# nash169/manifold-gp

Hardware: AMD Instinct MI355X
Metric: CG-solve wall-time + SpMV HBM GB/s, N=60k RMNIST graph (higher is better)
Workload: dtype f32; 1 GPU; C3 RMNIST-like N=60000 d=784 k=50 nu=2 randomwalk; nodes=60000, edges=1777442, nnz_padded=3667592, rhs_columns=1, system=A = I + noise*outputscale*Q, Q=(2nu/kappa^2 I + L)^nu x D, solver=CG on A (Chronopoulos-Gear, one hipGraph per solve)

## Files before the change

include/mgp_hip.h:

```cpp
#ifndef MGP_HIP_H
#define MGP_HIP_H

#include <stddef.h>
#include <stdint.h>

#ifdef __cplusplus
extern "C" {
#endif

#define MGP_OK 0
#define MGP_ERR_ARG (-1)
#define MGP_ERR_WORKSPACE (-2)
#define MGP_ERR_UNSUPPORTED (-3)
#define MGP_ERR_NOT_CONVERGED (-4)
#define MGP_ERR_KNN_AMBIGUOUS (-5)
#define MGP_ERR_TIMEOUT (-6)

#define MGP_PAD 4

int mgp_version(void);
int mgp_device_info(int* cu_count, int* wave_size, size_t* hbm_bytes);

size_t mgp_knn_workspace_bytes(int64_t N, int64_t n, int d, int k);
int mgp_knn_search(const float* db, int64_t N, int d, const float* q, int64_t n, int k,
// ... 129 lines not shown

typedef struct {
  float tol;
  int32_t max_iter;
  int32_t min_iter;
  int32_t stop_mode;
  int32_t check_every;
  int32_t use_graph;
  int32_t max_refine;
} mgp_cg_params_t;

size_t mgp_cg_workspace_bytes(const mgp_operator_t* op, int C);
int mgp_cg_set_decide_in_update(int on);
int mgp_cg_set_complex_shift(int on);
int mgp_cg_plan_is_complex_shift(void* plan);
int mgp_cg_set_fold_update(int on);
int mgp_cg_plan_is_folded(void* plan);
int mgp_cg_set_reduce_once(int on);
int mgp_cg_set_update_quads(int on);
int mgp_cg_set_poll_spin(int spins);
int mgp_cg_set_init_free(int on);
int mgp_cg_plan_create(const mgp_operator_t* op, int C, const float* minv,
                       const mgp_cg_params_t* params, void* work, size_t work_bytes, void* stream,
                       void** plan_out);
int mgp_cg_plan_solve(void* plan, const float* B, float* X, int32_t* iters, float* resid,
                      int32_t* status);
int mgp_cg_plan_rebind(void* plan, const mgp_operator_t* op, const float* minv);
float* mgp_cg_plan_x(void* plan);
double* mgp_cg_plan_x64(void* plan);
int mgp_cg_plan_last_applies(void* plan);
// ... 179 lines not shown
```

manifold_gp_amd/_lib.py:

```python
import ctypes
import os
import threading
from ctypes import (POINTER, Structure, byref, c_double, c_float, c_int, c_int32, c_int64, c_size_t,
                    c_uint64, c_void_p)

import torch

_HERE = os.path.dirname(os.path.abspath(__file__))
LIB_PATH = os.path.join(_HERE, "libmgp_hip.so")
_LIB = None
_LOCK = threading.Lock()

MGP_ERRORS = {
    -1: "MGP_ERR_ARG (null pointer / bad size / bad enum)",
    -2: "MGP_ERR_WORKSPACE (work buffer too small)",
    -3: "MGP_ERR_UNSUPPORTED",
    -4: "MGP_ERR_NOT_CONVERGED",
    -5: "MGP_ERR_KNN_AMBIGUOUS",
}


class MgpError(RuntimeError):
    def __init__(self, fn, code):
        self.code = code
# ... 57 lines not shown
    "mgp_spmm_dot_blocks_csr": (c_int, [POINTER(CsrT), c_int]),
    "mgp_spmm_set_tile_mode": (c_int, [c_int]),
    "mgp_spmm_set_tile_loop_mode": (c_int, [c_int]),
    "mgp_spmm_set_tile_small_mode": (c_int, [c_int]),
    "mgp_spmm_set_tile_wide_mode": (c_int, [c_int]),
    "mgp_spmm_set_dict_mode": (c_int, [c_int]),
    "mgp_spmm_set_mt_mode": (c_int, [c_int]),
    "mgp_spmm_kernel_choice": (c_int, [POINTER(CsrT), c_int, c_int, c_int64]),
    "mgp_spmm_mt_fill": (c_int, [c_int64, _P, _P, _P, _P, _P, _P, c_int64, _P, _P, _P]),
    "mgp_spmm_timing_begin": (c_int, [c_int]),
    "mgp_spmm_timing_end": (c_int, [POINTER(c_float), POINTER(c_int)]),
    "mgp_spmm_set_v4_mode": (c_int, [c_int]),
    "mgp_cg_set_decide_in_update": (c_int, [c_int]),
    "mgp_cg_set_complex_shift": (c_int, [c_int]),
    "mgp_cg_plan_is_complex_shift": (c_int, [_P]),
    "mgp_cg_set_fold_update": (c_int, [c_int]),
    "mgp_cg_plan_is_folded": (c_int, [_P]),
    "mgp_cg_set_reduce_once": (c_int, [c_int]),
    "mgp_cg_set_update_quads": (c_int, [c_int]),
    "mgp_cg_set_poll_spin": (c_int, [c_int]),
    "mgp_cg_set_init_free": (c_int, [c_int]),
    "mgp_host_symeig": (c_int, [c_int, _P, _P, _P]),
    "mgp_lanczos_set_bound_mode": (c_int, [c_int]),
    "mgp_blz_workspace_bytes": (c_size_t, [c_int64, c_int, c_int]),
    "mgp_blz_begin": (c_int, [_P, c_int64, c_int, c_int, _P, c_size_t, _P]),
    "mgp_blz_q": (c_void_p, [c_int64, c_int, c_int, c_int, _P, c_size_t]),
    "mgp_blz_step": (c_int, [_P, c_int64, c_int, c_int, c_int, _P, c_size_t, _P]),
    "mgp_blz_end": (c_int, [c_int64, c_int, c_int, POINTER(c_float), POINTER(c_float), _P, c_size_t, _P]),
    "mgp_lanczos_tridiag_block_workspace_bytes": (c_size_t, [POINTER(OperatorT), c_int, c_int]),
    "mgp_lanczos_tridiag_block": (c_int, [POINTER(OperatorT), _P, c_int, c_int, POINTER(c_float), POINTER(c_float), _P,
# ... 237 lines not shown
```

manifold_gp_amd/csrc/cg.hip:

```cpp
#include <math.h>
#include <chrono>
#include <mutex>
#include <new>
#include <vector>
#include <string.h>
#include <algorithm>
#include "mgp_common.h"
#include "mgp_internal.h"
#include "cg_rule.h"
#include "cg_policy.h"
#include "cg_handoff.h"

namespace {

#ifndef MGP_LAB_UPD
#define MGP_LAB_UPD 0
#endif

typedef float mgp_cg_v4f __attribute__((ext_vector_type(4)));

struct CgArgs {
  int64_t n;
  int C, TC, TS;
  float *x, *r, *u, *w, *p, *s;
// ... 647 lines not shown
  const mgp_cg_v4f* y4;
  const float* pd4;
  int nbs4;
  float sigma;
  float* pd_g;
  float* sc;
};

__device__ __forceinline__ float2 cx_mul(float2 a, float2 b) { return make_float2(a.x * b.x - a.y * b.y, a.x * b.y + a.y * b.x); }
__device__ __forceinline__ float2 cx_div(float2 a, float2 b) {
  const float d = b.x * b.x + b.y * b.y;
  if (!(d > 0.f)) return make_float2(0.f, 0.f);
  return make_float2((a.x * b.x + a.y * b.y) / d, (a.y * b.x - a.x * b.y) / d);
}

__global__ __launch_bounds__(kBlock) void cx_init_kernel(CgArgs a, CxArgs c, const float* __restrict__ B) {
  __shared__ float sh_o[kBlock / 64];
  const int tid = threadIdx.x, lane = tid & 63, wave = tid >> 6;
  const int lb = mgp_xcd_block(blockIdx.x, gridDim.x);
  const int64_t r0 = (int64_t)lb * a.rows_per_block;
  int64_t r1 = r0 + a.rows_per_block;
  if (r1 > a.n) r1 = a.n;
  if (blockIdx.x == 0 && tid == 0) { a.state[0] = 0; a.state[1] = 0; a.state[2] = 0; }
  float g = 0.f;
  for (int64_t r = r0 + tid; r < r1; r += kBlock) {
    const float b = B[r];
    c.z[r] = make_float2(0.f, 0.f);
    c.r[r] = make_float2(b, 0.f);
    c.p[r] = make_float2(0.f, 0.f);
    c.s[r] = make_float2(0.f, 0.f);
    c.u4[r] = mgp_cg_v4f{b, 0.f, b, 0.f};
    c.w4[r] = mgp_cg_v4f{b, 0.f, 0.f, b};
    a.x[r] = 0.f;
    g = fmaf(b, b, g);
  }
  g = mgp_wave_sum(g);
  if (lane == 0) sh_o[wave] = g;
  __syncthreads();
  if (tid == 0) {
    const float t = (sh_o[0] + sh_o[1]) + (sh_o[2] + sh_o[3]);
    float* dst = c.pd_g + 4 * (int64_t)lb;
    dst[0] = t; dst[1] = 0.f; dst[2] = t; dst[3] = t;
  }
}

__global__ __launch_bounds__(kBlock) void cx_update_kernel(CgArgs a, CxArgs c) {
  __shared__ float sh_w[kBlock / 64][8];
  __shared__ float sh_o[kBlock / 64][4];
  __shared__ int sh_state[2];
  const int tid = threadIdx.x, lane = tid & 63, wave = tid >> 6;
  const int st_it = a.state[0], st_done = a.state[1];
  const int lb = mgp_xcd_block(blockIdx.x, gridDim.x);
  const int64_t r0 = (int64_t)lb * a.rows_per_block;
  int64_t r1 = r0 + a.rows_per_block;
  if (r1 > a.n) r1 = a.n;
  float t[8] = {0.f, 0.f, 0.f, 0.f, 0.f, 0.f, 0.f, 0.f};
  mgp_cg_v4f gv[2][kC1GammaSlots];
#pragma unroll
  for (int h = 0; h < 2; ++h) {
#pragma unroll
// ... 66 lines not shown
  const CgStop st = cg_stop(1, 0, a.max_iter + 1, a.tol, it, rel);
  const int done = st.done;
  if (blockIdx.x == 0 && tid == 0) {
    c.sc[4 * par + 0] = gamma.x; c.sc[4 * par + 1] = gamma.y;
    c.sc[4 * par + 2] = alpha.x; c.sc[4 * par + 3] = alpha.y;
    if (it == 1) c.sc[8] = bb;
    a.resid[0] = rel;
    if (done) cg_publish(a.state, a.host_state, a.host_resid, &rel, 1, it, st.status);
  }
  if (done) return;
  float ngr = 0.f, ngi = 0.f, nrr = 0.f, nee = 0.f;
  constexpr int U = 4;
  const int64_t rf = r0 + tid;
  for (int64_t rb = rf; rb < r1; rb += (int64_t)U * kBlock) {
    float2 uo[U], po[U], so[U], zo[U];
    mgp_cg_v4f yo[U];
#pragma unroll
    for (int k = 0; k < U; ++k) {
      const int64_t r = rb + (int64_t)k * kBlock;
      const int64_t rc = r < r1 ? r : rf;
      uo[k] = c.r[rc]; po[k] = c.p[rc]; so[k] = c.s[rc]; zo[k] = c.z[rc]; yo[k] = c.y4[rc];
    }
#pragma unroll
    for (int k = 0; k < U; ++k) {
      const int64_t r = rb + (int64_t)k * kBlock;
      if (r < r1) {
        const float2 u = uo[k];
        const float2 w = make_float2(u.x - c.sigma * yo[k].y, u.y + c.sigma * yo[k].x);
        const float e = u.x + c.sigma * yo[k].y;
        const float2 bp = cx_mul(beta, po[k]), bs = cx_mul(beta, so[k]);
        const float2 pn = make_float2(u.x + bp.x, u.y + bp.y);
        const float2 sn = make_float2(w.x + bs.x, w.y + bs.y);
        const float2 ap = cx_mul(alpha, pn), as = cx_mul(alpha, sn);
        const float2 zn = make_float2(zo[k].x + ap.x, zo[k].y + ap.y);
        const float2 rn = make_float2(u.x - as.x, u.y - as.y);
        c.p[r] = pn; c.s[r] = sn; c.z[r] = zn; c.r[r] = rn;
        a.x[r] = zo[k].x;
        c.u4[r] = mgp_cg_v4f{rn.x, rn.y, rn.x, rn.y};
        c.w4[r] = mgp_cg_v4f{rn.x, rn.y, rn.y, rn.x};
        ngr += rn.x * rn.x - rn.y * rn.y;
        ngi += 2.f * rn.x * rn.y;
        nrr += rn.x * rn.x + rn.y * rn.y;
        nee = fmaf(e, e, nee);
      }
    }
  }
  ngr = mgp_wave_sum(ngr); ngi = mgp_wave_sum(ngi); nrr = mgp_wave_sum(nrr); nee = mgp_wave_sum(nee);
  if (lane == 0) { sh_o[wave][0] = ngr; sh_o[wave][1] = ngi; sh_o[wave][2] = nrr; sh_o[wave][3] = nee; }
  __syncthreads();
  if (tid == 0) {
    float* dst = c.pd_g + 4 * ((int64_t)par * a.nbv + lb);
    dst[0] = (sh_o[0][0] + sh_o[1][0]) + (sh_o[2][0] + sh_o[3][0]);
    dst[1] = (sh_o[0][1] + sh_o[1][1]) + (sh_o[2][1] + sh_o[3][1]);
    dst[2] = (sh_o[0][2] + sh_o[1][2]) + (sh_o[2][2] + sh_o[3][2]);
// ... 152 lines not shown
  hipGraph_t graph_first = nullptr;
  hipGraphExec_t exec_first = nullptr;
  hipGraphNode_t init_node = nullptr;
  bool has_graph = false, has_first = false;
  int chunk = 0, len_first = 0;
  int last_need = 0;
  const float* patched_rhs = nullptr;
  int solves = 0;
  int64_t last_solve_ns = 0;
  int marker_seq = 0;
  bool graphs_tried = false;
  bool rebound = false;
  bool decide_in_update = false;
  CxArgs cxa{};
  mgp_operator_t opB{};
  char first_record[MGP_SPMM_RECORD_BYTES] = {};
  int32_t* host_state = nullptr;
  float* host_resid = nullptr;
  float* host_true_rel = nullptr;
  float* dev_true_rel = nullptr;
};

CgKnobs g_knobs;

CgShape cg_shape(const mgp_operator_t* op, int C, int world, bool is_dist, bool has_minv, int stop_mode) {
  CgShape sh{};
  sh.n = op->L.n; sh.world = world; sh.is_dist = is_dist; sh.C = C;
  sh.nb_loc = mgp_spmm_dot_blocks_for(&op->L, C);
  sh.nb4 = (C == 1 && !is_dist) ? mgp_spmm_dot_blocks_for(&op->L, 4) : 0;
  sh.has_minv = has_minv; sh.has_pre = op->pre != nullptr; sh.has_post = op->post != nullptr;
// ... 31 lines not shown

MgpCgStep fold_step(const CgPlan* pl) {
  const CgArgs& a = pl->args;
  MgpCgStep cs{};
  cs.r = a.r; cs.x = a.x; cs.p = a.p; cs.s = a.s; cs.us = a.us; cs.pre = a.pre;
  cs.pd_rr = a.pd_rr; cs.pd_delta = a.pd_delta; cs.nbs = a.nbs;
  cs.blk = a.gamma_old; cs.state = a.state; cs.host_state = a.host_state; cs.host_resid = a.host_resid; cs.arrive = a.arrive;
  cs.tol = a.tol; cs.max_iter = a.max_iter; cs.min_iter = a.min_iter; cs.stop_mode = a.stop_mode;
  return cs;
}

int enqueue_body(CgPlan* pl, hipStream_t st, bool decide_last = false) {
  if (pl->ch.fold)
    return mgp_operator_apply_cgstep(&pl->op, pl->args.us ? pl->args.us : pl->args.r, false, nullptr, fold_step(pl), decide_last,
                                     pl->buf.op_work, pl->buf.op_work_bytes, st);
  if (pl->ch.cx) {
    MGP_TRY(mgp_operator_apply_dist(&pl->opB, nullptr, reinterpret_cast<const float*>(pl->cxa.u4), nullptr, 4,
                                    const_cast<float*>(reinterpret_cast<const float*>(pl->cxa.y4)),
                                    reinterpret_cast<const float*>(pl->cxa.w4), pl->buf.pd4, pl->cxa.nbs4, pl->args.state + 1,
                                    pl->args.state, pl->buf.op_work4, pl->buf.op_work4_bytes, st));
    hipLaunchKernelGGL(cx_update_kernel, dim3(pl->args.nbv), dim3(kBlock), 0, st, pl->args, pl->cxa);
    MGP_LAUNCH_CHECK();
    return MGP_OK;
  }
  MGP_TRY(mgp_operator_apply_dist(&pl->op, pl->is_dist ? &pl->dist : nullptr, pl->args.u, pl->args.us, pl->C,
                                  pl->args.w, pl->args.u, pl->buf.pd_delta, pl->nb_loc, pl->args.state + 1,
                                  pl->args.state, pl->buf.op_work, pl->buf.op_work_bytes, st));
  if (pl->ch.c1_family) {
    launch_update_c1(pl, st, decide_last);
  } else {
    if (pl->args.tot) {
      hipLaunchKernelGGL(cg_reduce_kernel, dim3((unsigned)mgp_cdiv(pl->C, 4), 3), dim3(kBlock), 0, st, pl->args);
      MGP_LAUNCH_CHECK();
    }
    if (pl->ch.upd_quads) hipLaunchKernelGGL(cg_update_q_kernel<kBlock>, dim3(pl->args.nbv), dim3(kBlock), 0, st, pl->args);
    else hipLaunchKernelGGL(cg_update_kernel, dim3(pl->args.nbv), dim3(kBlock), 0, st, pl->args);
// ... 207 lines not shown
  a.tol = prm.tol; a.max_iter = prm.max_iter; a.min_iter = prm.min_iter; a.stop_mode = prm.stop_mode;
  (void)hipMemsetAsync(a.state, 0, (16 + kStampWords) * sizeof(int), pl->stream);
  MGP_HIP_TRY(hipMemsetAsync(a.arrive, 0, 9 * 32 * sizeof(int), pl->stream));
  if (b.cz) {
    CxArgs& cx = pl->cxa;
    cx.z = reinterpret_cast<float2*>(b.cz); cx.r = reinterpret_cast<float2*>(b.cr);
    cx.p = reinterpret_cast<float2*>(b.cp); cx.s = reinterpret_cast<float2*>(b.cs);
    cx.u4 = reinterpret_cast<mgp_cg_v4f*>(b.u4); cx.w4 = reinterpret_cast<mgp_cg_v4f*>(b.w4);
    cx.y4 = reinterpret_cast<const mgp_cg_v4f*>(b.y4);
    cx.pd4 = b.pd4; cx.pd_g = b.pd_g; cx.sc = b.sc;
  }
  if (ch.cx) {
    pl->opB = cx_operator(op);
    pl->cxa.nbs4 = sh.nb4;
    pl->cxa.sigma = sqrtf(sh.noise_scale);
    MGP_HIP_TRY(hipMemsetAsync(pl->cxa.sc, 0, 64 * sizeof(float), pl->stream));
  }
  const size_t rbytes = (((size_t)C * sizeof(float)) + 63) & ~size_t(63);
  if (!host_block_acquire(64 + 2 * rbytes, &pl->host_block)) { delete pl; return (int)hipErrorOutOfMemory; }
  char* hb = static_cast<char*>(pl->host_block.p);
  pl->host_state = reinterpret_cast<int32_t*>(hb);
  pl->host_resid = reinterpret_cast<float*>(hb + 64);
  pl->host_true_rel = reinterpret_cast<float*>(hb + 64 + rbytes);
  hipError_t e = hipHostGetDevicePointer((void**)&a.host_state, pl->host_state, 0);
  if (e == hipSuccess) e = hipHostGetDevicePointer((void**)&a.host_resid, pl->host_resid, 0);
  if (e == hipSuccess) e = hipHostGetDevicePointer((void**)&pl->dev_true_rel, pl->host_true_rel, 0);
  if (e != hipSuccess) { host_block_release(pl->host_block, pl->stream); delete pl; return (int)e; }
  memset(hb, 0, 64 + 2 * rbytes);

  *plan_out = pl;
  return MGP_OK;
}

extern "C" int mgp_cg_set_init_free(int on) { g_knobs.init_free = on ? 1 : 0; return MGP_OK; }
extern "C" int mgp_cg_set_poll_spin(int spins) { g_knobs.poll_spin = spins < 0 ? 0 : spins; return MGP_OK; }
extern "C" int mgp_cg_set_reduce_once(int on) { g_knobs.reduce_once = on == 2 ? 2 : (on ? 1 : 0); return MGP_OK; }
extern "C" int mgp_cg_set_update_quads(int on) { g_knobs.update_quads = on ? 1 : 0; return MGP_OK; }
extern "C" int mgp_cg_set_complex_shift(int on) { const int prev = g_knobs.complex_shift; g_knobs.complex_shift = on ? 1 : 0; return prev; }
extern "C" int mgp_cg_set_decide_in_update(int on) { const int prev = g_knobs.decide_in_update; g_knobs.decide_in_update = on ? 1 : 0; return prev; }

extern "C" int mgp_cg_set_fold_update(int on) { const int prev = g_knobs.fold_update; g_knobs.fold_update = on == 2 ? 2 : (on ? 1 : 0); return prev; }

extern "C" int mgp_cg_plan_is_folded(void* plan) {
  CgPlan* pl = static_cast<CgPlan*>(plan);
  return pl && pl->ch.fold ? 1 : 0;
}

extern "C" int mgp_cg_plan_is_complex_shift(void* plan) {
  CgPlan* pl = static_cast<CgPlan*>(plan);
  return pl && pl->ch.cx ? 1 : 0;
}

extern "C" int mgp_cg_plan_create(const mgp_operator_t* op, int C, const float* minv,
                                  const mgp_cg_params_t* params, void* work, size_t work_bytes,
                                  void* stream, void** plan_out) {
  return plan_create_impl(op, C, minv, params, nullptr, work, work_bytes, stream, plan_out);
}

extern "C" int mgp_cg_plan_rebind(void* plan, const mgp_operator_t* op, const float* minv) {
  CgPlan* pl = static_cast<CgPlan*>(plan);
  if (!pl || !op) return MGP_ERR_ARG;
  if (pl->poisoned || pl->is_dist) return MGP_ERR_UNSUPPORTED;
  const mgp_operator_t& o = pl->op;
  const bool same = op->L.n == o.L.n && op->L.ncols == o.L.ncols && op->nu == o.nu && op->form == o.form &&
                    (op->form != 3 || ((op->obs_w != nullptr) == (o.obs_w != nullptr))) &&
                    (op->pre != nullptr) == (o.pre != nullptr) && (op->post != nullptr) == (o.post != nullptr) &&
                    (minv != nullptr) == (pl->args.minv != nullptr) &&
                    (op->L.tile_ptr != nullptr) == (o.L.tile_ptr != nullptr) && op->L.tile_rows == o.L.tile_rows &&
                    op->L.tile_max_cols == o.L.tile_max_cols && op->L.tile_max_entries == o.L.tile_max_entries &&
                    (op->L.tile_rowptr != nullptr) == (o.L.tile_rowptr != nullptr) &&
                    (op->L.tile_vals != nullptr) == (o.L.tile_vals != nullptr) &&
                    (op->L.tile_rowid != nullptr) == (o.L.tile_rowid != nullptr) &&
                    (op->L.mt_img != nullptr) == (o.L.mt_img != nullptr) && op->L.mt_tiles == o.L.mt_tiles &&
                    op->L.mt_steps == o.L.mt_steps && op->L.spmv_lanes == o.L.spmv_lanes &&
                    mgp_spmm_dot_blocks_for(&op->L, pl->C) == pl->nb_loc &&
                    (!pl->ch.fold || op->pre == op->post);
  if (!same) return MGP_ERR_UNSUPPORTED;
  if (pl->ch.cx) {
    const float cc = op->noise * op->scale;
    if (!(cc > 0.f)) return MGP_ERR_UNSUPPORTED;
    pl->opB = cx_operator(op);
    if (mgp_spmm_dot_blocks_for(&pl->opB.L, 4) != pl->cxa.nbs4) return MGP_ERR_UNSUPPORTED;
    pl->cxa.sigma = sqrtf(cc);
  }
  pl->op = mgp_operator_copy(op);
  pl->args.minv = minv;
  pl->args.pre = op->pre;
  pl->rebound = true;
  return MGP_OK;
}

extern "C" size_t mgp_cg_dist_workspace_bytes(const mgp_operator_t* op_local, int C, int world) {
  if (!op_local || C <= 0 || C > kMaxC || op_local->L.n <= 0 || world < 1 || !mgp_spmv_lanes_ok(op_local->L.spmv_lanes)) return 0;
  return cg_bytes(op_local, C, world, true);
}

extern "C" int mgp_cg_plan_create_dist(const mgp_operator_t* op_local, int C, const float* minv,
// ... 6 lines not shown

static int run_cg(CgPlan* pl, const float* rhs, float* Xcopy) {
  hipStream_t st = pl->stream;
  const size_t nc = (size_t)pl->args.n * pl->C;
  pl->host_state[1] = 0;
  pl->host_state[3] = 0;
  *reinterpret_cast<volatile uint64_t*>(pl->host_state + 8) = 0;
  bool first = true;
  const auto t_begin = std::chrono::steady_clock::now();
  if (pl->rebound) refresh_graphs(pl);
  if (pl->solves++ >= 1 && !pl->graphs_tried) capture_graphs(pl);
  if (pl->has_first && !patch_first_rhs(pl, rhs)) pl->has_first = false;
  int eager_done = 0;
  if (!pl->has_first) {
    if (pl->ch.cx) {
      hipLaunchKernelGGL(cx_init_kernel, dim3(pl->args.nbv), dim3(kBlock), 0, st, pl->args, pl->cxa, rhs);
      MGP_LAUNCH_CHECK();
    } else if (pl->ch.init_free) {
      MGP_TRY(enqueue_first_body(pl, st, rhs, false));
      eager_done = 1;
    } else {
      hipLaunchKernelGGL(cg_init_kernel, dim3(pl->args.nbv), dim3(kBlock), 0, st, pl->args, rhs);
      MGP_LAUNCH_CHECK();
    }
  }
  int guard = 0;
  for (;;) {
    const bool launched_first = first && pl->has_first;
    if (launched_first) {
      ++pl->marker_seq;
      MGP_HIP_TRY(hipGraphLaunch(pl->exec_first, st));
// ... 203 lines not shown
```

manifold_gp_amd/csrc/cg_policy.h:

```cpp
#pragma once
#include <stdint.h>
#include <stddef.h>
#include "mgp_hip.h"
#include "mgp_arena.h"

constexpr int kBlock = 256;
constexpr int kMaxC = 256;
constexpr int kMaxGridVec = 512;
constexpr int kMaxPartials = 4096;
constexpr int kReduceOnceAbove = 16;
constexpr int kC1GammaSlots = 2;
constexpr int kC1DeltaSlots = 16;
constexpr int kCxDeltaSlots = 16;
#ifdef MGP_STAMP
constexpr size_t kStampWords = 1024 + 8192;
#else
constexpr size_t kStampWords = 0;
#endif

struct CgKnobs {
  int complex_shift = 1;
  int reduce_once = 1;
  int update_quads = 1;
  int poll_spin = 64;
  int init_free = 1;
  int decide_in_update = 1;
  int fold_update = 1;
};

struct CgShape {
  int64_t n;
  int world;
  bool is_dist;
  int C, nb_loc, nb4;
  bool has_minv, has_pre, has_post;
  int form, nu;
  float noise_scale;
  int stop_mode;
  bool tile_plan;
  bool pre_is_post;
  int tile_rows;
};
// ... 101 lines not shown
```

manifold_gp_amd/csrc/mgp_internal.h:

```cpp
#pragma once
#include <stddef.h>
#include <string.h>
#include <vector>
#include "mgp_hip.h"

inline mgp_operator_t mgp_operator_copy(const mgp_operator_t* op) {
  mgp_operator_t o;
  memcpy(&o, op, offsetof(mgp_operator_t, obs_w));
  o.obs_w = op->form == 3 ? op->obs_w : nullptr;
  return o;
}

inline bool mgp_spmv_lanes_ok(int lanes) {
  return lanes == 0 || lanes == 4 || lanes == 8 || lanes == 16 || lanes == 32 || lanes == 64;
}

#define MGP_SPMM_RECORD_BYTES 512
struct MgpFirst {
  float* copy_x;
  float* dot2_partials;
  int tick_reset;
  void* record;
};
struct MgpSpmmOpts {
// ... 17 lines not shown
  float* host_resid;
  int* arrive;
  float tol;
  int max_iter, min_iter, stop_mode;
  float dcoef;
  int dgamma;
};
int mgp_spmm_cgstep(const mgp_csr_t* L, const float* T, float a, float b, const float* post, float co, const MgpCgStep& cs,
                    bool decide, void* stream);
int mgp_spmm_cgstep_fits(const mgp_csr_t* L);
int mgp_operator_apply_cgstep(const mgp_operator_t* op, const float* in, bool first, void* record, const MgpCgStep& cs, bool decide,
                              void* work, size_t work_bytes, void* stream);
int mgp_spmm_fused_opts(const mgp_csr_t* L, const float* X, int C, float* Y, float a, float b, const float* pre,
                        const float* post, const float* base, float cb, float co, const float* dotw, float* dot_partials,
                        const MgpSpmmOpts& opts, void* stream);
int mgp_spmm_patch_node(void* exec, void* node, const void* record, const float* old_ptr, const float* new_ptr);
int mgp_operator_apply_first(const mgp_operator_t* op, const float* rhs, float* r_copy, float* Y, float* dot_partials,
                             float* dot2_partials, int* state, void* record, void* work, size_t work_bytes, void* stream);
int mgp_tile_plan(const mgp_csr_t* L);

int mgp_spmm_dot_blocks_for(const mgp_csr_t* L, int C);

int mgp_operator_apply_ex(const mgp_operator_t* op, const float* X, int C, float* Y, const float* dotw,
                          float* dot_partials, const int* skip, int* tick, void* work, size_t work_bytes,
                          void* stream);

int mgp_operator_apply_ex2(const mgp_operator_t* op, const float* X, const float* Xs, int C, float* Y,
                           const float* dotw, float* dot_partials, const int* skip, int* tick, void* work,
                           size_t work_bytes, void* stream);

// ... 60 lines not shown
```

manifold_gp_amd/csrc/operator.hip:

```cpp
#include <rccl/rccl.h>
#include "mgp_common.h"
#include "mgp_internal.h"

namespace {

struct Hooks {
  const float* dotw;
  float* dot_partials;
  const int* skip;
  int* tick;
  float* copy_x;
  void* record;
  float* dot2_partials;
  int tick_reset;
};

}

int mgp_dist_allgather_f32(const MgpDist* d, float* buf, int64_t count_per_rank, void* stream) {
  ncclResult_t r = ncclAllGather(buf + (int64_t)d->rank * count_per_rank, buf, (size_t)count_per_rank, ncclFloat,
                                 static_cast<ncclComm_t>(d->comm), mgp_stream(stream));
  return r == ncclSuccess ? MGP_OK : 1000 + (int)r;
}

// ... 85 lines not shown
  switch (op->form) {
    case 0:
      return q2_chain(op, d, nb_loc, X, Xs, C, Y, nullptr, 0.f, 1.f, t0, t1, &hk, stream);
    case 2:
      return q2_chain(op, d, nb_loc, X, Xs, C, Y, X, 1.f, op->noise, t0, t1, &hk, stream);
    case 3:
      return q2_chain(op, d, nb_loc, X, Xs, C, Y, X, 1.f, op->noise, t0, t1, &hk, stream, op->obs_w);
    case 1:
      MGP_TRY(q2_chain(op, d, nb_loc, X, Xs, C, ua, X, 1.f, -op->noise, t0, t1, &hk_mid, stream));
      MGP_TRY(q2_chain(op, d, nb_loc, ua, nullptr, C, ub, X, 1.f, -op->noise, t0, t1, &hk_mid, stream));
      return q2_chain(op, d, nb_loc, ub, nullptr, C, Y, nullptr, 0.f, 1.f, t0, t1, &hk, stream);
  }
  return MGP_ERR_ARG;
}

int mgp_operator_apply_first(const mgp_operator_t* op, const float* rhs, float* r_copy, float* Y, float* dot_partials,
                             float* dot2_partials, int* state, void* record, void* work, size_t work_bytes, void* stream) {
  MGP_TRY(check_op(op));
  if (!rhs || !r_copy || !Y || !dot_partials || !dot2_partials || !state || rhs == Y) return MGP_ERR_ARG;
  if (op->form != 0 && op->form != 2) return MGP_ERR_UNSUPPORTED;
  if (!work || work_bytes < 4 * mgp_align((size_t)op->L.n * sizeof(float))) return MGP_ERR_WORKSPACE;
  MgpArena ar(work, work_bytes);
  const size_t nc = (size_t)op->L.n;
  float* t0 = ar.take<float>(nc);
  float* t1 = ar.take<float>(nc);
  if (!ar.ok()) return MGP_ERR_WORKSPACE;
  const float* rv = op->nu == 1 ? rhs : r_copy;
  Hooks hk{rv, dot_partials, nullptr, state, r_copy, record, dot2_partials, 1};
  if (op->form == 0) return q2_chain(op, nullptr, 0, rhs, nullptr, 1, Y, nullptr, 0.f, 1.f, t0, t1, &hk, stream);
  return q2_chain(op, nullptr, 0, rhs, nullptr, 1, Y, rv, 1.f, op->noise, t0, t1, &hk, stream);
// ... 206 lines not shown
```

manifold_gp_amd/csrc/spmm.hip:

```cpp
#include <string.h>
#include <atomic>
#include <type_traits>
#include "mgp_common.h"
#include "mgp_internal.h"
#include "cg_rule.h"
#include "cg_handoff.h"
#include <hip/hip_ext.h>
#include <vector>

namespace {

constexpr int kBlock = 256;
constexpr int kMaxGrid = 4096;

struct SpmmArgs {
  int64_t n;
  const int32_t* rowptr;
  const int32_t* col;
  const float* vals;
  const float* diag;
  const float* X;
  float* Y;
  int C;
  float a, b;
// ... 959 lines not shown
  }
  if (p.tick && blockIdx.x == 0 && tid == 0 && !skipv) *p.tick = tickv + 1;
  if (p.dot_partials) {
    __syncthreads();
    float* red = tile_lds;
    if (sub < C4) *reinterpret_cast<mgp_v4f*>(red + (size_t)(tid >> 2) * C + 4 * sub) = dsum;
    __syncthreads();
    if (tid < C) {
      float sacc = 0.f;
      for (int r = 0; r < TR; ++r) sacc += red[r * C + tid];
      p.dot_partials[(int64_t)lb * C + tid] = sacc;
    }
  }
}

constexpr int kWideCap = 1024;
constexpr int kWideRQ = 16;

template <bool PRE, bool CBV>
__global__ __launch_bounds__(256, 2) void spmm_tile_wide_kernel(SpmmArgs p, TileArgs t, int dict_cap) {
  extern __shared__ __attribute__((aligned(16))) float tile_lds[];
  constexpr int BS = 256, TR = 64;
  const int skipv = p.skip ? *p.skip : 0;
  const int tickv = (p.tick && blockIdx.x == 0) ? *p.tick : 0;
  const int lb = mgp_xcd_block(blockIdx.x, gridDim.x);
  const int tid = threadIdx.x, sub = tid & 3;
  const int C = p.C, C4 = C >> 2;
  mgp_v4f* __restrict__ xl = reinterpret_cast<mgp_v4f*>(tile_lds);
  const mgp_v4f* __restrict__ X4 = reinterpret_cast<const mgp_v4f*>(p.X);
  const float* __restrict__ prev = p.pre;
// ... 545 lines not shown
  return (int)mgp_cdiv(ntiles, tpb);
}

static int tile_small_window(const mgp_csr_t* L) {
  const int max_q = L->tile_max_entries >> 2;
  const long budget = 40448 - (long)L->tile_max_cols * 16;
  long w = budget > 0 ? budget / 16 / 256 * 256 : 0;
  if (w < 1024) w = 1024;
  if (w > max_q) w = (max_q + 255) / 256 * 256;
  return (int)(w > 0 ? w : 256);
}
static size_t tile_small_lds_bytes(const mgp_csr_t* L, int C) {
  const size_t max_q = (size_t)(L->tile_max_entries >> 2), w = (size_t)tile_small_window(L);
  size_t b = ((size_t)L->tile_max_cols + (max_q < w ? max_q : w)) * 16;
  const size_t red = (size_t)64 * C * sizeof(float);
  return b > red ? b : red;
}

static int tile_wide_cap(const mgp_csr_t* L) {
  int cap = (L->tile_max_cols + 63) / 64 * 64;
  if (cap > kWideCap) cap = kWideCap;
  if (cap < 64) cap = 64;
  return cap;
}
static size_t tile_wide_lds_bytes(const mgp_csr_t* L) {
  const size_t b = (size_t)tile_wide_cap(L) * 64;
  return b > 4096 ? b : 4096;
}

static int dict_nv(int C) { return (C + 63) / 64; }
// ... 385 lines not shown
  const TileArgs ta = tile_args(L, pl.tiles_per_block, 0);
  const dim3 grid(pl.grid), block(256);
  hipStream_t st = mgp_stream(stream);
  auto step = [&](auto ds, auto one) {
    constexpr int DS = decltype(ds)::value;
    constexpr bool ONE = decltype(one)::value;
    if (decide) hipLaunchKernelGGL((spmv_tile_cgstep_kernel<256, DS, true, ONE>), grid, block, pl.lds, st, p, ta, cs);
    else hipLaunchKernelGGL((spmv_tile_cgstep_kernel<256, DS, false, ONE>), grid, block, pl.lds, st, p, ta, cs);
  };
  if (cs.nbs <= 4 * 256) { if (pl.one_tile) step(IntC<4>{}, std::true_type{}); else step(IntC<4>{}, std::false_type{}); }
  else { if (pl.one_tile) step(IntC<16>{}, std::true_type{}); else step(IntC<16>{}, std::false_type{}); }
  MGP_LAUNCH_CHECK();
  return MGP_OK;
}

extern "C" int mgp_spmm_fused(const mgp_csr_t* L, const float* X, int C, float* Y, float a, float b,
                              const float* pre, const float* post, const float* base, float cb,
                              float co, const float* dotw, float* dot_partials, void* stream) {
  return mgp_spmm_fused_opts(L, X, C, Y, a, b, pre, post, base, cb, co, dotw, dot_partials, MgpSpmmOpts{}, stream);
}

__global__ void scale_rows_kernel(const float* __restrict__ s, const float* __restrict__ x,
                                  float* __restrict__ y, int64_t n, int C) {
  int64_t total = n * C;
  for (int64_t i = blockIdx.x * (int64_t)blockDim.x + threadIdx.x; i < total;
       i += (int64_t)gridDim.x * blockDim.x)
    y[i] = s[i / C] * x[i];
}

extern "C" int mgp_laplacian_matmul(const mgp_csr_t* L, const float* dsqrt, const float* dinvsqrt,
// ... 84 lines not shown
```

manifold_gp_amd/solvers.py:

```python
import ctypes
import math
import warnings

import torch

from . import _lib
from ._compat import settings
from ._lib import CgParamsT, LanczosParamsT, check, lib, ptr, stream


RELABEL_SOLVES = [True]
CHAIN_SOLVE_MIN_C = [8]


class CgPlan:

    def __init__(self, desc, C, tol=None, max_iter=None, min_iter=None, stop_mode=None, jacobi=None,
                 check_every=0, use_graph=True, refine=0):
        self.C = int(C)
        self._xout = None
        desc = self._bind(desc)
        dev = desc.data.graph.device
        stop_mode = settings.cg_stop_mode.value() if stop_mode is None else stop_mode
        self.params = CgParamsT(
# ... 43 lines not shown
            return False
        self.minv = minv
        return True

    @property
    def applies(self):
        return self._applies_fn(self.handle)

    @property
    def resid(self):
        return list(self._resid)

    @property
    def complex_shift(self):
        return bool(lib().mgp_cg_plan_is_complex_shift(self.handle))

    @property
    def folded(self):
        return bool(lib().mgp_cg_plan_is_folded(self.handle))

    def solution_view(self):
        if self._xview is None:
            off = int(lib().mgp_cg_plan_x(self.handle)) - self.work.data_ptr()
            nb = self.desc.n * self.C * 4
            self._xview = self.work[off:off + nb].view(torch.float32).view(self.desc.n, self.C)
        return self._xview

    def solution64_view(self):
        p = lib().mgp_cg_plan_x64(self.handle)
        if not p or self.params.max_refine <= 0:
# ... 498 lines not shown
```

Measured before the change: 3856 GB/s (algorithmic SpMV bytes inside the CG solve).

## Add two-column complex-pair SpMV kernel for the complex-shift CG path

Adds a tile SpMV kernel that works on the complex residual stored as interleaved float2 pairs. It computes the four real/imag dot partials in its epilogue. Before, the complex-shift path ran a 4-column SpMV on duplicated u4/w4 vectors. The CG update and init kernels no longer write those duplicated vectors, which cuts gather, write and streaming traffic per iteration. The new path is on by default when the tile-small plan and the LDS budget allow it. It adds a new kernel with its own LDS windowing, plus a fallback when the plan does not fit.

```diff
diff --git a/include/mgp_hip.h b/include/mgp_hip.h
--- a/include/mgp_hip.h
+++ b/include/mgp_hip.h
@@ -167,6 +167,8 @@
 int mgp_cg_set_decide_in_update(int on);
 int mgp_cg_set_complex_shift(int on);
 int mgp_cg_plan_is_complex_shift(void* plan);
+int mgp_cg_set_cx_pair(int on);
+int mgp_cg_plan_is_cx_pair(void* plan);
 int mgp_cg_set_fold_update(int on);
 int mgp_cg_plan_is_folded(void* plan);
 int mgp_cg_set_reduce_once(int on);
diff --git a/manifold_gp_amd/_lib.py b/manifold_gp_amd/_lib.py
--- a/manifold_gp_amd/_lib.py
+++ b/manifold_gp_amd/_lib.py
@@ -95,6 +95,8 @@
     "mgp_cg_set_decide_in_update": (c_int, [c_int]),
     "mgp_cg_set_complex_shift": (c_int, [c_int]),
     "mgp_cg_plan_is_complex_shift": (c_int, [_P]),
+    "mgp_cg_set_cx_pair": (c_int, [c_int]),
+    "mgp_cg_plan_is_cx_pair": (c_int, [_P]),
     "mgp_cg_set_fold_update": (c_int, [c_int]),
     "mgp_cg_plan_is_folded": (c_int, [_P]),
     "mgp_cg_set_reduce_once": (c_int, [c_int]),
diff --git a/manifold_gp_amd/csrc/cg.hip b/manifold_gp_amd/csrc/cg.hip
--- a/manifold_gp_amd/csrc/cg.hip
+++ b/manifold_gp_amd/csrc/cg.hip
@@ -685,6 +685,7 @@
   return make_float2((a.x * b.x + a.y * b.y) / d, (a.y * b.x - a.x * b.y) / d);
 }
 
+template <bool PAIR>
 __global__ __launch_bounds__(kBlock) void cx_init_kernel(CgArgs a, CxArgs c, const float* __restrict__ B) {
   __shared__ float sh_o[kBlock / 64];
   const int tid = threadIdx.x, lane = tid & 63, wave = tid >> 6;
@@ -700,8 +701,10 @@
     c.r[r] = make_float2(b, 0.f);
     c.p[r] = make_float2(0.f, 0.f);
     c.s[r] = make_float2(0.f, 0.f);
-    c.u4[r] = mgp_cg_v4f{b, 0.f, b, 0.f};
-    c.w4[r] = mgp_cg_v4f{b, 0.f, 0.f, b};
+    if (!PAIR) {
+      c.u4[r] = mgp_cg_v4f{b, 0.f, b, 0.f};
+      c.w4[r] = mgp_cg_v4f{b, 0.f, 0.f, b};
+    }
     a.x[r] = 0.f;
     g = fmaf(b, b, g);
   }
@@ -715,6 +718,7 @@
   }
 }
 
+template <bool PAIR>
 __global__ __launch_bounds__(kBlock) void cx_update_kernel(CgArgs a, CxArgs c) {
   __shared__ float sh_w[kBlock / 64][8];
   __shared__ float sh_o[kBlock / 64][4];
@@ -811,12 +815,14 @@
   const int64_t rf = r0 + tid;
   for (int64_t rb = rf; rb < r1; rb += (int64_t)U * kBlock) {
     float2 uo[U], po[U], so[U], zo[U];
-    mgp_cg_v4f yo[U];
+    float2 yo[U];
 #pragma unroll
     for (int k = 0; k < U; ++k) {
       const int64_t r = rb + (int64_t)k * kBlock;
       const int64_t rc = r < r1 ? r : rf;
-      uo[k] = c.r[rc]; po[k] = c.p[rc]; so[k] = c.s[rc]; zo[k] = c.z[rc]; yo[k] = c.y4[rc];
+      uo[k] = c.r[rc]; po[k] = c.p[rc]; so[k] = c.s[rc]; zo[k] = c.z[rc];
+      if (PAIR) yo[k] = reinterpret_cast<const float2*>(c.y4)[rc];
+      else { const mgp_cg_v4f y = c.y4[rc]; yo[k] = make_float2(y.x, y.y); }
     }
 #pragma unroll
     for (int k = 0; k < U; ++k) {
@@ -833,8 +839,10 @@
         const float2 rn = make_float2(u.x - as.x, u.y - as.y);
         c.p[r] = pn; c.s[r] = sn; c.z[r] = zn; c.r[r] = rn;
         a.x[r] = zo[k].x;
-        c.u4[r] = mgp_cg_v4f{rn.x, rn.y, rn.x, rn.y};
-        c.w4[r] = mgp_cg_v4f{rn.x, rn.y, rn.y, rn.x};
+        if (!PAIR) {
+          c.u4[r] = mgp_cg_v4f{rn.x, rn.y, rn.x, rn.y};
+          c.w4[r] = mgp_cg_v4f{rn.x, rn.y, rn.y, rn.x};
+        }
         ngr += rn.x * rn.x - rn.y * rn.y;
         ngi += 2.f * rn.x * rn.y;
         nrr += rn.x * rn.x + rn.y * rn.y;
@@ -1017,6 +1025,7 @@
   bool decide_in_update = false;
   CxArgs cxa{};
   mgp_operator_t opB{};
+  bool cx_pair = false;
   char first_record[MGP_SPMM_RECORD_BYTES] = {};
   int32_t* host_state = nullptr;
   float* host_resid = nullptr;
@@ -1078,12 +1087,20 @@
   if (pl->ch.fold)
     return mgp_operator_apply_cgstep(&pl->op, pl->args.us ? pl->args.us : pl->args.r, false, nullptr, fold_step(pl), decide_last,
                                      pl->buf.op_work, pl->buf.op_work_bytes, st);
+  if (pl->ch.cx && pl->cx_pair) {
+    MGP_TRY(mgp_operator_apply_cx_pair(&pl->opB, reinterpret_cast<const float*>(pl->cxa.r),
+                                       const_cast<float*>(reinterpret_cast<const float*>(pl->cxa.y4)), pl->buf.pd4,
+                                       pl->args.state + 1, pl->args.state, st));
+    hipLaunchKernelGGL(cx_update_kernel<true>, dim3(pl->args.nbv), dim3(kBlock), 0, st, pl->args, pl->cxa);
+    MGP_LAUNCH_CHECK();
+    return MGP_OK;
+  }
   if (pl->ch.cx) {
     MGP_TRY(mgp_operator_apply_dist(&pl->opB, nullptr, reinterpret_cast<const float*>(pl->cxa.u4), nullptr, 4,
                                     const_cast<float*>(reinterpret_cast<const float*>(pl->cxa.y4)),
                                     reinterpret_cast<const float*>(pl->cxa.w4), pl->buf.pd4, pl->cxa.nbs4, pl->args.state + 1,
                                     pl->args.state, pl->buf.op_work4, pl->buf.op_work4_bytes, st));
-    hipLaunchKernelGGL(cx_update_kernel, dim3(pl->args.nbv), dim3(kBlock), 0, st, pl->args, pl->cxa);
+    hipLaunchKernelGGL(cx_update_kernel<false>, dim3(pl->args.nbv), dim3(kBlock), 0, st, pl->args, pl->cxa);
     MGP_LAUNCH_CHECK();
     return MGP_OK;
   }
@@ -1321,6 +1338,7 @@
     pl->opB = cx_operator(op);
     pl->cxa.nbs4 = sh.nb4;
     pl->cxa.sigma = sqrtf(sh.noise_scale);
+    pl->cx_pair = knobs.cx_pair != 0 && mgp_spmm_cx_pair_fits(&pl->opB.L) != 0;
     MGP_HIP_TRY(hipMemsetAsync(pl->cxa.sc, 0, 64 * sizeof(float), pl->stream));
   }
   const size_t rbytes = (((size_t)C * sizeof(float)) + 63) & ~size_t(63);
@@ -1344,6 +1362,7 @@
 extern "C" int mgp_cg_set_reduce_once(int on) { g_knobs.reduce_once = on == 2 ? 2 : (on ? 1 : 0); return MGP_OK; }
 extern "C" int mgp_cg_set_update_quads(int on) { g_knobs.update_quads = on ? 1 : 0; return MGP_OK; }
 extern "C" int mgp_cg_set_complex_shift(int on) { const int prev = g_knobs.complex_shift; g_knobs.complex_shift = on ? 1 : 0; return prev; }
+extern "C" int mgp_cg_set_cx_pair(int on) { const int prev = g_knobs.cx_pair; g_knobs.cx_pair = on ? 1 : 0; return prev; }
 extern "C" int mgp_cg_set_decide_in_update(int on) { const int prev = g_knobs.decide_in_update; g_knobs.decide_in_update = on ? 1 : 0; return prev; }
 
 extern "C" int mgp_cg_set_fold_update(int on) { const int prev = g_knobs.fold_update; g_knobs.fold_update = on == 2 ? 2 : (on ? 1 : 0); return prev; }
@@ -1356,6 +1375,11 @@
 extern "C" int mgp_cg_plan_is_complex_shift(void* plan) {
   CgPlan* pl = static_cast<CgPlan*>(plan);
   return pl && pl->ch.cx ? 1 : 0;
+}
+
+extern "C" int mgp_cg_plan_is_cx_pair(void* plan) {
+  CgPlan* pl = static_cast<CgPlan*>(plan);
+  return pl && pl->ch.cx && pl->cx_pair ? 1 : 0;
 }
 
 extern "C" int mgp_cg_plan_create(const mgp_operator_t* op, int C, const float* minv,
@@ -1386,8 +1410,10 @@
   if (pl->ch.cx) {
     const float cc = op->noise * op->scale;
     if (!(cc > 0.f)) return MGP_ERR_UNSUPPORTED;
-    pl->opB = cx_operator(op);
-    if (mgp_spmm_dot_blocks_for(&pl->opB.L, 4) != pl->cxa.nbs4) return MGP_ERR_UNSUPPORTED;
+    const mgp_operator_t ob = cx_operator(op);
+    if (mgp_spmm_dot_blocks_for(&ob.L, 4) != pl->cxa.nbs4) return MGP_ERR_UNSUPPORTED;
+    if (pl->cx_pair && !mgp_spmm_cx_pair_fits(&ob.L)) return MGP_ERR_UNSUPPORTED;
+    pl->opB = ob;
     pl->cxa.sigma = sqrtf(cc);
   }
   pl->op = mgp_operator_copy(op);
@@ -1424,7 +1450,8 @@
   int eager_done = 0;
   if (!pl->has_first) {
     if (pl->ch.cx) {
-      hipLaunchKernelGGL(cx_init_kernel, dim3(pl->args.nbv), dim3(kBlock), 0, st, pl->args, pl->cxa, rhs);
+      if (pl->cx_pair) hipLaunchKernelGGL(cx_init_kernel<true>, dim3(pl->args.nbv), dim3(kBlock), 0, st, pl->args, pl->cxa, rhs);
+      else hipLaunchKernelGGL(cx_init_kernel<false>, dim3(pl->args.nbv), dim3(kBlock), 0, st, pl->args, pl->cxa, rhs);
       MGP_LAUNCH_CHECK();
     } else if (pl->ch.init_free) {
       MGP_TRY(enqueue_first_body(pl, st, rhs, false));
diff --git a/manifold_gp_amd/csrc/cg_policy.h b/manifold_gp_amd/csrc/cg_policy.h
--- a/manifold_gp_amd/csrc/cg_policy.h
+++ b/manifold_gp_amd/csrc/cg_policy.h
@@ -26,6 +26,7 @@
   int init_free = 1;
   int decide_in_update = 1;
   int fold_update = 1;
+  int cx_pair = 1;
 };
 
 struct CgShape {
diff --git a/manifold_gp_amd/csrc/mgp_internal.h b/manifold_gp_amd/csrc/mgp_internal.h
--- a/manifold_gp_amd/csrc/mgp_internal.h
+++ b/manifold_gp_amd/csrc/mgp_internal.h
@@ -55,6 +55,11 @@
 int mgp_spmm_fused_opts(const mgp_csr_t* L, const float* X, int C, float* Y, float a, float b, const float* pre,
                         const float* post, const float* base, float cb, float co, const float* dotw, float* dot_partials,
                         const MgpSpmmOpts& opts, void* stream);
+int mgp_spmm_cx_pair(const mgp_csr_t* L, const float* U, float* Y2, float a, float b, const float* post, float co,
+                     float* dot_partials, const int* skip, int* tick, void* stream);
+int mgp_spmm_cx_pair_fits(const mgp_csr_t* L);
+int mgp_operator_apply_cx_pair(const mgp_operator_t* op, const float* U, float* Y2, float* dot_partials, const int* skip, int* tick,
+                               void* stream);
 int mgp_spmm_patch_node(void* exec, void* node, const void* record, const float* old_ptr, const float* new_ptr);
 int mgp_operator_apply_first(const mgp_operator_t* op, const float* rhs, float* r_copy, float* Y, float* dot_partials,
                              float* dot2_partials, int* state, void* record, void* work, size_t work_bytes, void* stream);
diff --git a/manifold_gp_amd/csrc/operator.hip b/manifold_gp_amd/csrc/operator.hip
--- a/manifold_gp_amd/csrc/operator.hip
+++ b/manifold_gp_amd/csrc/operator.hip
@@ -123,6 +123,14 @@
   return MGP_ERR_ARG;
 }
 
+int mgp_operator_apply_cx_pair(const mgp_operator_t* op, const float* U, float* Y2, float* dot_partials, const int* skip, int* tick,
+                               void* stream) {
+  MGP_TRY(check_op(op));
+  if (op->form != 0 || op->nu != 1 || op->pre) return MGP_ERR_UNSUPPORTED;
+  const float tau = 2.0f * (float)op->nu / (op->kappa * op->kappa);
+  return mgp_spmm_cx_pair(&op->L, U, Y2, tau, 1.0f, op->post, 1.f * op->scale, dot_partials, skip, tick, stream);
+}
+
 int mgp_operator_apply_first(const mgp_operator_t* op, const float* rhs, float* r_copy, float* Y, float* dot_partials,
                              float* dot2_partials, int* state, void* record, void* work, size_t work_bytes, void* stream) {
   MGP_TRY(check_op(op));
diff --git a/manifold_gp_amd/csrc/spmm.hip b/manifold_gp_amd/csrc/spmm.hip
--- a/manifold_gp_amd/csrc/spmm.hip
+++ b/manifold_gp_amd/csrc/spmm.hip
@@ -997,6 +997,141 @@
   }
 }
 
+__device__ __forceinline__ mgp_v2f pair_products(mgp_v4f vv, mgp_v2f a0, mgp_v2f a1, mgp_v2f a2, mgp_v2f a3) {
+  const mgp_v2f vlo = mgp_v2f{vv.x, vv.y}, vhi = mgp_v2f{vv.z, vv.w};
+  mgp_v2f lo = pk_mul_lo(vlo, a0);
+  lo = pk_fma_hi(vlo, a1, lo);
+  lo = pk_fma_lo(vhi, a2, lo);
+  lo = pk_fma_hi(vhi, a3, lo);
+  return lo;
+}
+
+__global__ __launch_bounds__(256, 4) void spmm_tile_pair_kernel(SpmmArgs p, TileArgs t) {
+  extern __shared__ __attribute__((aligned(16))) float tile_lds[];
+  constexpr int BS = 256, TR = 64, NQ = 4;
+  const int skipv = p.skip ? *p.skip : 0;
+  const int tickv = (p.tick && blockIdx.x == 0) ? *p.tick : 0;
+  const int lb = mgp_xcd_block(blockIdx.x, gridDim.x);
+  const int tid = threadIdx.x, sub = tid & 3;
+  mgp_v2f* __restrict__ xl = reinterpret_cast<mgp_v2f*>(tile_lds);
+  mgp_v2f* __restrict__ part = xl + t.max_cols;
+  const mgp_v2f* __restrict__ X2 = reinterpret_cast<const mgp_v2f*>(p.X);
+  const int32_t* __restrict__ rowptr = t.rowptr_t ? t.rowptr_t : p.rowptr;
+  const float* __restrict__ vals = t.vals_t ? t.vals_t : p.vals;
+  const int32_t* __restrict__ tile_ptr = t.tile_ptr;
+  const uint32_t* __restrict__ tile_cols = reinterpret_cast<const uint32_t*>(t.tile_cols);
+  const uint16_t* __restrict__ lid = t.lid;
+  mgp_v4f dsum = mgp_v4f{0.f, 0.f, 0.f, 0.f};
+  const int64_t t0 = (int64_t)lb * t.tiles_per_block;
+  const int64_t t1 = t0 + t.tiles_per_block < t.ntiles ? t0 + t.tiles_per_block : t.ntiles;
+  for (int64_t tile = t0; tile < t1; ++tile) {
+    const int64_t r0 = tile * TR;
+    const int64_t r1 = r0 + TR < p.n ? r0 + TR : p.n;
+    const int e0 = rowptr[r0], e1 = rowptr[r1];
+    const int dp = tile_ptr[tile];
+    const int D = tile_ptr[tile + 1] - dp;
+    const int qb = e0 >> 2, Q = (e1 - e0) >> 2;
+    if (skipv) return;
+    unsigned c[NQ];
+#pragma unroll
+    for (int k = 0; k < NQ; ++k) {
+      const int j = tid + k * BS;
+      c[k] = (unsigned)tile_cols[j < D ? dp + j : 0];
+    }
+    __builtin_amdgcn_sched_barrier(0);
+    mgp_v4f v[NQ];
+    mgp_v4h l[NQ];
+#pragma unroll
+    for (int k = 0; k < NQ; ++k) {
+      const int q = tid + k * BS;
+      const int qi = q < Q ? qb + q : 0;
+      v[k] = *reinterpret_cast<const mgp_v4f*>(vals + 4 * (int64_t)qi);
+      l[k] = *reinterpret_cast<const mgp_v4h*>(lid + 4 * (int64_t)qi);
+    }
+    __builtin_amdgcn_sched_barrier(0);
+    mgp_v2f g[NQ];
+#pragma unroll
+    for (int k = 0; k < NQ; ++k) g[k] = X2[(int64_t)c[k]];
+    __builtin_amdgcn_sched_barrier(0);
+    const int64_t row = r0 + (tid >> 2);
+    const bool valid = row < r1;
+    const int64_t pr = valid ? row : r0;
+    const int64_t rr = t.rowid ? (int64_t)t.rowid[pr] : pr;
+    const int64_t grr = rr + p.goff;
+    const int rs = rowptr[pr], re = rowptr[pr + 1];
+    const float e_diag = p.diag[rr];
+    const float l_post = p.post ? p.post[grr] : 1.f;
+    const mgp_v2f e_x = X2[grr];
+    __builtin_amdgcn_sched_barrier(0);
+#pragma unroll
+    for (int k = 0; k < NQ; ++k) {
+      const int j = tid + k * BS;
+      if (j < D) xl[j] = g[k];
+    }
+    for (int j = tid + NQ * BS; j < D; j += BS) xl[j] = X2[(int64_t)tile_cols[dp + j]];
+    mgp_v2f acc = mgp_v2f{0.f, 0.f};
+    const int W = t.part_window;
+    for (int w0 = 0; w0 == 0 || w0 < Q; w0 += W) {
+      const int w1 = Q < w0 + W ? Q : w0 + W;
+      __syncthreads();
+#pragma unroll
+      for (int k = 0; k < NQ; ++k) {
+        const int q = tid + k * BS;
+        if (q >= w0 && q < w1) {
+          const mgp_v2f a0 = xl[l[k].x], a1 = xl[l[k].y], a2 = xl[l[k].z], a3 = xl[l[k].w];
+          part[q - w0] = pair_products(v[k], a0, a1, a2, a3);
+        }
+      }
+      {
+        int q = tid + NQ * BS;
+        if (q < w0) q += (w0 - q + BS - 1) / BS * BS;
+        for (; q < w1; q += BS) {
+          const mgp_v4f vv = *reinterpret_cast<const mgp_v4f*>(vals + 4 * (int64_t)(qb + q));
+          const mgp_v4h ll = *reinterpret_cast<const mgp_v4h*>(lid + 4 * (int64_t)(qb + q));
+          const mgp_v2f a0 = xl[ll.x], a1 = xl[ll.y], a2 = xl[ll.z], a3 = xl[ll.w];
+          part[q - w0] = pair_products(vv, a0, a1, a2, a3);
+        }
+      }
+      __syncthreads();
+      {
+        int i = (rs >> 2) - qb + sub;
+        if (i < w0) i += (w0 - i + 3) / 4 * 4;
+        int e = (re >> 2) - qb;
+        if (e > w1) e = w1;
+        for (; i + 4 < e; i += 8) {
+          const mgp_v2f a0 = part[i - w0], a1 = part[i + 4 - w0];
+          acc.x += a0.x; acc.y += a0.y;
+          acc.x += a1.x; acc.y += a1.y;
+        }
+        for (; i < e; i += 4) {
+          const mgp_v2f a0 = part[i - w0];
+          acc.x += a0.x; acc.y += a0.y;
+        }
+      }
+    }
+    acc.x = mgp_quad_sum(acc.x); acc.y = mgp_quad_sum(acc.y);
+    if (valid && sub == 0) {
+      mgp_v2f y;
+      y.x = p.co * ((p.a * e_x.x + p.b * (e_diag * e_x.x - acc.x)) * l_post) + 0.f;
+      y.y = p.co * ((p.a * e_x.y + p.b * (e_diag * e_x.y - acc.y)) * l_post) + 0.f;
+      *reinterpret_cast<mgp_v2f*>(p.Y + 2 * grr) = y;
+      dsum.x = fmaf(e_x.x, y.x, dsum.x); dsum.y = fmaf(e_x.y, y.y, dsum.y);
+      dsum.z = fmaf(e_x.y, y.x, dsum.z); dsum.w = fmaf(e_x.x, y.y, dsum.w);
+    }
+    if (tile + 1 < t1) __syncthreads();
+  }
+  if (p.tick && blockIdx.x == 0 && tid == 0 && !skipv) *p.tick = tickv + 1;
+  __syncthreads();
+  float* red = tile_lds;
+  if (sub == 0) *reinterpret_cast<mgp_v4f*>(red + (size_t)(tid >> 2) * 4) = dsum;
+  __syncthreads();
+  if (tid < 4) {
+    float sacc = 0.f;
+    for (int r = 0; r < TR; ++r) sacc += red[r * 4 + tid];
+    p.dot_partials[(int64_t)lb * 4 + tid] = sacc;
+  }
+}
+
 constexpr int kWideCap = 1024;
 constexpr int kWideRQ = 16;
 
@@ -1572,6 +1707,21 @@
   const size_t max_q = (size_t)(L->tile_max_entries >> 2), w = (size_t)tile_small_window(L);
   size_t b = ((size_t)L->tile_max_cols + (max_q < w ? max_q : w)) * 16;
   const size_t red = (size_t)64 * C * sizeof(float);
+  return b > red ? b : red;
+}
+
+static int tile_pair_window(const mgp_csr_t* L) {
+  const int max_q = L->tile_max_entries >> 2;
+  const long budget = 40448 - (long)L->tile_max_cols * 8;
+  long w = budget > 0 ? budget / 8 / 256 * 256 : 0;
+  if (w < 1024) w = 1024;
+  if (w > max_q) w = (max_q + 255) / 256 * 256;
+  return (int)(w > 0 ? w : 256);
+}
+static size_t tile_pair_lds_bytes(const mgp_csr_t* L) {
+  const size_t max_q = (size_t)(L->tile_max_entries >> 2), w = (size_t)tile_pair_window(L);
+  const size_t b = ((size_t)L->tile_max_cols + (max_q < w ? max_q : w)) * 8;
+  const size_t red = (size_t)64 * 4 * sizeof(float);
   return b > red ? b : red;
 }
 
@@ -1987,6 +2137,28 @@
   return MGP_OK;
 }
 
+int mgp_spmm_cx_pair_fits(const mgp_csr_t* L) {
+  if (!L) return 0;
+  const SpmmPlan pl = spmm_plan(L, 4, 0, true);
+  return pl.err == MGP_OK && pl.family == SpmmFamily::TileSmall && tile_pair_lds_bytes(L) <= 65536 - 64;
+}
+
+int mgp_spmm_cx_pair(const mgp_csr_t* L, const float* U, float* Y2, float a, float b, const float* post, float co,
+                     float* dot_partials, const int* skip, int* tick, void* stream) {
+  if (!L || !L->rowptr || !L->col || !L->vals || !L->diag || !U || !Y2 || !dot_partials || L->n <= 0) return MGP_ERR_ARG;
+  if (U == Y2) return MGP_ERR_ARG;
+  if (((reinterpret_cast<uintptr_t>(U) | reinterpret_cast<uintptr_t>(Y2)) & 7) != 0) return MGP_ERR_ARG;
+  const SpmmPlan pl = spmm_plan(L, 4, 0, true);
+  if (pl.err != MGP_OK) return pl.err;
+  if (pl.family != SpmmFamily::TileSmall || tile_pair_lds_bytes(L) > 65536 - 64) return MGP_ERR_UNSUPPORTED;
+  SpmmArgs p{L->n, L->rowptr, L->col, L->vals, L->diag, U, Y2, 2, a, b, nullptr, post, nullptr, 0.f, co,
+             nullptr, dot_partials, 0, skip, tick, 0, nullptr, nullptr, 0, nullptr};
+  const TileArgs ta = tile_args(L, pl.tiles_per_block, tile_pair_window(L));
+  hipLaunchKernelGGL(spmm_tile_pair_kernel, dim3(pl.grid), dim3(256), tile_pair_lds_bytes(L), mgp_stream(stream), p, ta);
+  MGP_LAUNCH_CHECK();
+  return MGP_OK;
+}
+
 extern "C" int mgp_spmm_fused(const mgp_csr_t* L, const float* X, int C, float* Y, float a, float b,
                               const float* pre, const float* post, const float* base, float cb,
                               float co, const float* dotw, float* dot_partials, void* stream) {
diff --git a/manifold_gp_amd/solvers.py b/manifold_gp_amd/solvers.py
--- a/manifold_gp_amd/solvers.py
+++ b/manifold_gp_amd/solvers.py
@@ -81,6 +81,10 @@
     @property
     def complex_shift(self):
         return bool(lib().mgp_cg_plan_is_complex_shift(self.handle))
+
+    @property
+    def complex_pair(self):
+        return bool(lib().mgp_cg_plan_is_cx_pair(self.handle))
 
     @property
     def folded(self):
```

New measurement: 3835 GB/s (algorithmic SpMV bytes inside the CG solve), median of 2. About the same (-0.5%).
